# apache/horaedb

Measured on NVIDIA H100. Metric: scanned rows/s, higher is better.
Workload: dtype f64

## Files before the change

horaedb_b200/csrc/snappy.cu:

```cuda
#include "kernels.h"
#include "chunk_scratch.h"

#include <cstdlib>
#include <cstring>

#define SNP_FN __device__ __forceinline__
#define snp_shfl(v, src) __shfl_sync(0xffffffffu, (v), (src))
#define snp_shfl_up(v, d) __shfl_up_sync(0xffffffffu, (v), (d))
#define snp_ballot(p) __ballot_sync(0xffffffffu, (p))
#define snp_any(p) __any_sync(0xffffffffu, (p))
#define snp_syncwarp() __syncwarp()
#define snp_ldg8(p) __ldg(p)
#define snp_ldg64(p) __ldg(p)
#define snp_funnel_r(lo, hi, sh) __funnelshift_r((lo), (hi), (sh))
#define snp_byte_perm(a, b, s) __byte_perm((a), (b), (s))
#define snp_ffs(x) __ffs(x)
#define snp_set_err(err, code) atomicExch((err), (code))
namespace horae {
namespace snp {
__device__ __forceinline__ uint32_t snp_ldcg32(const uint32_t* p) {
  uint32_t v;
  asm volatile("ld.global.cg.u32 %0, [%1];" : "=r"(v) : "l"(p));
  return v;
}
__device__ __forceinline__ uint8_t snp_ldcg8(const uint8_t* p) {
  uint32_t v;
  asm volatile("ld.global.cg.u8 %0, [%1];" : "=r"(v) : "l"(p));
  return uint8_t(v);
}
}
}
#include "snappy_core.h"

namespace horae {
namespace k {

namespace {

using namespace horae::snp;
constexpr int kWarpsPerCta = 4;

__device__ __forceinline__ void init_tag_tables(uint8_t* s_csz, uint32_t* s_lut) {
  for (uint32_t t = threadIdx.x; t < 256; t += kWarpsPerCta * 32) { s_csz[t] = uint8_t(elem_csize(t)); s_lut[t] = elem_lut(t); }
  __syncthreads();
}

__global__ void __launch_bounds__(kWarpsPerCta * 32, 8) snappy_pages_kernel(const __grid_constant__ SnappyJob J) {
  __shared__ WarpSmem s_w[kWarpsPerCta];
  __shared__ uint32_t s_lut[256];
  __shared__ uint8_t s_csz[256];
  init_tag_tables(s_csz, s_lut);
  const int lane = threadIdx.x & 31, wid = threadIdx.x >> 5;
  WarpSmem& sm = s_w[wid];
  bulk_init(sm, lane);
  uint32_t phase = 0;
  const uint32_t nsel = J.d_nsel ? *J.d_nsel : J.nsel;
  const uint32_t nchunks = nsel * uint32_t(J.ncols);
  for (;;) {
    uint32_t c = 0;
    if (lane == 0) c = atomicAdd(J.ticket, 1u);
    c = __shfl_sync(0xffffffffu, c, 0);
    if (c >= nchunks) return;
    const uint32_t si = J.lpt ? J.lpt[c % nsel] : c % nsel;
    const int ci = J.order[c / nsel];
    RgSel rs = J.sel[si];
    SstDev sst = J.ssts[rs.sst];
    const ChunkDev* chunks = sst.chunks + size_t(rs.rg) * sst.ncols;
    ChunkDev ch = chunks[J.col_from_cols ? J.cols[ci].col : J.col[ci]];
    if (ch.codec != CODEC_SNAPPY) continue;
    if (ch.stored && J.skip_stored[ci]) continue;
    uint8_t* dst = J.scratch + (J.fixed_stride ? rs.scratch_off + uint64_t(J.region[ci]) * J.fixed_stride
                                               : chunk_scratch_off(rs, chunks, J.cols, ci));
    for (int p = ch.dict_uncomp ? -1 : 0; p < int(ch.num_pages); p++) {
      const uint8_t* src;
      uint32_t n, ulen, stop_at = 0xffffffffu;
      uint64_t advance;
      bool compressed = true;
      if (p < 0) {
        src = sst.bytes + ch.dict_payload_off; n = ch.dict_comp; ulen = ch.dict_uncomp;
        advance = dict_scratch(ch.codec, ch.phys, ch.dict_uncomp);
      } else {
        const PageDev pg = sst.pages[ch.first_page + p];
        const PageStream ps = page_stream(pg);
        src = sst.bytes + pg.payload_off + ps.skip; n = ps.comp; ulen = ps.out;
        compressed = ps.compressed;
        if (J.partial[ci]) {
          const uint32_t w = (ch.phys == 1 || ch.phys == 4) ? 4u : 8u;
          stop_at = 16u + (rs.num_rows + 7u) / 8u + 8u + rs.out_row * w;
        }
        advance = page_body_scratch(ch.codec, pg) + page_image_scratch(pg);
      }
      if (compressed) snappy_page(src, n, dst, ulen, stop_at, sm, phase, s_csz, s_lut, lane, J.err);
      dst += advance;
    }
  }
}

__global__ void __launch_bounds__(kWarpsPerCta * 32, 8) snappy_raw_kernel(const RawPage* __restrict__ pages, uint32_t n, unsigned int* ticket, int* err) {
  __shared__ WarpSmem s_w[kWarpsPerCta];
  __shared__ uint32_t s_lut[256];
  __shared__ uint8_t s_csz[256];
  init_tag_tables(s_csz, s_lut);
  const int lane = threadIdx.x & 31, wid = threadIdx.x >> 5;
  bulk_init(s_w[wid], lane);
  uint32_t phase = 0;
  for (;;) {
    uint32_t c = 0;
    if (lane == 0) c = atomicAdd(ticket, 1u);
    c = __shfl_sync(0xffffffffu, c, 0);
    if (c >= n) return;
    const RawPage pg = pages[c];
    snappy_page(pg.src, pg.comp_size, pg.dst, pg.uncomp_size, 0xffffffffu, s_w[wid], phase, s_csz, s_lut, lane, err);
  }
}

}

static uint32_t snappy_max_ctas() {
  static const int env = getenv("HORAE_SNAPPY_CTAS_PER_SM") ? atoi(getenv("HORAE_SNAPPY_CTAS_PER_SM")) : 0;
  int n = env > 0 ? env : 7;
  if (n > 8) n = 8;
  return uint32_t(kNumSMs) * uint32_t(n);
}

void snappy_raw_pages(const Launch& L, const RawPage* d_pages, uint32_t n, unsigned int* ticket, int* err) {
  if (!n) return;
  uint32_t ctas = (n + kWarpsPerCta - 1) / kWarpsPerCta;
  if (ctas > snappy_max_ctas()) ctas = snappy_max_ctas();
  snappy_raw_kernel<<<ctas, kWarpsPerCta * 32, 0, L.stream>>>(d_pages, n, ticket, err);
  L.tick();
}

void snappy_pages(const Launch& L, const SnappyJob& job, uint32_t max_chunks) {
  if (!max_chunks) return;
  uint32_t ctas = (max_chunks + kWarpsPerCta - 1) / kWarpsPerCta;
  if (ctas > snappy_max_ctas()) ctas = snappy_max_ctas();
  snappy_pages_kernel<<<ctas, kWarpsPerCta * 32, 0, L.stream>>>(job);
  L.tick();
}

void snappy_chunks(const Launch& L, const SstDev* ssts, const RgSel* sel, uint32_t nsel, const ColSel* cols, int ncolsel,
                   uint8_t* scratch, unsigned int* ticket, int* err) {
  if (!nsel || !ncolsel) return;
  SnappyJob J;
  std::memset(&J, 0, sizeof(J));
  J.ssts = ssts; J.sel = sel; J.d_nsel = nullptr; J.nsel = nsel; J.cols = cols; J.ncols = ncolsel;
  J.scratch = scratch; J.ticket = ticket; J.err = err; J.fixed_stride = 0;
  for (int i = 0; i < ncolsel && i < kSnappyMaxCols; i++) J.order[i] = uint8_t(i);
  J.col_from_cols = 1;
  snappy_pages(L, J, nsel * uint32_t(ncolsel));
}

}
}
```

horaedb_b200/csrc/snappy_core.h:

```cpp
#pragma once
#include <cstdint>

#ifndef SNP_STAT
#define SNP_STAT(counter, amount)
#endif

namespace horae {
namespace snp {

constexpr int kWin = 256;
constexpr int kWinPad = 16;
constexpr int kRing = 4096;
constexpr int kHist = 2048;
constexpr int kLevels = 5;
constexpr uint32_t kExit = 0xff;
constexpr uint32_t kRestage = kWin - 80;
constexpr uint32_t kFlushAt = 512;
constexpr uint64_t kFill = 0xfcfcfcfcfcfcfcfcull;

constexpr int kStage = 448;
constexpr uint32_t kAhead = kRestage;
struct alignas(256) WarpSmem {
  uint64_t ring64[kRing / 8];
  uint8_t J[kLevels][kWin];
  alignas(16) uint8_t stage[2][kStage];
  uint64_t bar[2];
};
constexpr uint32_t kJOff = kRing;
constexpr uint32_t kStageOff = kRing + kLevels * kWin;
constexpr uint32_t kBarOff = kStageOff + 2 * kStage;
struct StageState {
  uint32_t phase;
  int cur;
  bool pf;
  int pf_start;
  uint32_t pf_bytes;
};

SNP_FN uint32_t elem_csize(uint32_t t) {
  const uint32_t kind = t & 3;
  if (kind == 0) { const uint32_t l = t >> 2; return l < 60 ? l + 2 : 255u; }
  return kind == 1 ? 2u : (kind == 2 ? 3u : 5u);
}
SNP_FN uint32_t elem_lut(uint32_t t) {
  const uint32_t kind = t & 3;
  uint32_t len, hdr, offhi = 0, is_lit = 0, long_lit = 0, msh = 0;
  if (kind == 0) {
    const uint32_t l = t >> 2;
    is_lit = 1; hdr = 1;
    if (l < 60) len = l + 1; else { len = 0; long_lit = 1; }
  } else if (kind == 1) { len = ((t >> 2) & 7) + 4; hdr = 2; offhi = t >> 5; msh = 24; }
  else if (kind == 2) { len = (t >> 2) + 1; hdr = 3; msh = 16; }
  else { len = (t >> 2) + 1; hdr = 5; msh = 0; }
  const uint32_t csz = long_lit ? 0u : hdr + (is_lit ? len : 0u);
  return len | (offhi << 8) | (is_lit << 16) | (long_lit << 17) | (msh << 18) | (csz << 24);
}

SNP_FN uint64_t funnel64(uint64_t lo, uint64_t hi, uint32_t sh_bits) {
  return (lo >> sh_bits) | ((hi << 1) << (63 - sh_bits));
}
SNP_FN uint64_t ld8_any(const uint8_t* p) {
  const uintptr_t a = reinterpret_cast<uintptr_t>(p);
  const uint64_t* q = reinterpret_cast<const uint64_t*>(a & ~uintptr_t(7));
  return funnel64(snp_ldg64(q), snp_ldg64(q + 1), uint32_t(a & 7) * 8);
}
SNP_FN uint64_t ld8_out(const uint8_t* p) {
  const uintptr_t a = reinterpret_cast<uintptr_t>(p);
  const uint32_t* q = reinterpret_cast<const uint32_t*>(a & ~uintptr_t(3));
  const uint32_t sh = uint32_t(a & 3) * 8;
  const uint32_t x = snp_ldcg32(q), y = snp_ldcg32(q + 1), z = snp_ldcg32(q + 2);
  return (uint64_t(snp_funnel_r(y, z, sh)) << 32) | snp_funnel_r(x, y, sh);
}
SNP_FN uint8_t* ring_bytes(WarpSmem& sm) { return reinterpret_cast<uint8_t*>(sm.ring64); }
SNP_FN uint64_t ring_ld8(const WarpSmem& sm, uint32_t x) {
  const uint32_t w = (x >> 3) & (kRing / 8 - 1);
  return funnel64(sm.ring64[w], sm.ring64[(w + 1) & (kRing / 8 - 1)], (x & 7) * 8);
}
SNP_FN uint64_t sm_ld8(const WarpSmem& sm, uint32_t a) {
  const uint32_t* w = reinterpret_cast<const uint32_t*>(&sm) + (a >> 2);
  const uint32_t sh = (a & 3) * 8;
  const uint32_t x = w[0], y = w[1], z = w[2];
  return (uint64_t(snp_funnel_r(y, z, sh)) << 32) | snp_funnel_r(x, y, sh);
}
SNP_FN uint64_t shfl64(uint64_t v, int src) {
  const uint32_t lo = snp_shfl(uint32_t(v), src);
  const uint32_t hi = snp_shfl(uint32_t(v >> 32), src);
  return (uint64_t(hi) << 32) | lo;
}
template <int I> SNP_FN uint32_t byte_of(uint32_t x) { return snp_byte_perm(x, 0u, 0x4440u + I); }
template <int I> SNP_FN uint32_t put_byte(uint32_t acc, uint32_t v) {
  return snp_byte_perm(acc, v, I == 0 ? 0x3214u : (I == 1 ? 0x3240u : (I == 2 ? 0x3410u : 0x4210u)));
}

#ifdef __CUDACC__
template <int I, int LV> SNP_FN uint32_t jt_get(const WarpSmem&, uint32_t smbase, uint32_t packed) {
  uint32_t v;
  asm volatile("ld.shared.u8 %0, [%1+%2];" : "=r"(v) : "r"(__byte_perm(packed, smbase, 0x7650u + I)), "n"(kJOff + LV * kWin));
  return v;
}
SNP_FN uint32_t sm_base(const WarpSmem& sm) { return uint32_t(__cvta_generic_to_shared(&sm)); }
#define SNP_ST_BYTE(i, v) asm volatile("{ .reg .pred p; setp.gt.u32 p, %2, " #i "; @p st.shared.u8 [%0+" #i "], %1; }" ::"r"(a), "r"(v), "r"(len) : "memory")
SNP_FN void store_elem(WarpSmem&, uint32_t smbase, uint32_t rb, uint64_t w, uint32_t len) {
  const uint32_t a = smbase + rb, lo = uint32_t(w), hi = uint32_t(w >> 32);
  asm volatile("st.shared.u8 [%0], %1;" ::"r"(a), "r"(lo) : "memory");
  SNP_ST_BYTE(1, lo >> 8); SNP_ST_BYTE(2, lo >> 16); SNP_ST_BYTE(3, lo >> 24);
  SNP_ST_BYTE(4, hi); SNP_ST_BYTE(5, hi >> 8); SNP_ST_BYTE(6, hi >> 16); SNP_ST_BYTE(7, hi >> 24);
}
#undef SNP_ST_BYTE
#else
template <int I, int LV> SNP_FN uint32_t jt_get(const WarpSmem& sm, uint32_t, uint32_t packed) { return sm.J[LV][(packed >> (8 * I)) & 0xffu]; }
SNP_FN uint32_t sm_base(const WarpSmem&) { return 0; }
SNP_FN void store_elem(WarpSmem& sm, uint32_t, uint32_t rb, uint64_t w, uint32_t len) {
  for (uint32_t i = 0; i < len; i++) reinterpret_cast<uint8_t*>(sm.ring64)[rb + i] = uint8_t(w >> (8 * i));
}
#endif
#ifdef __CUDACC__
SNP_FN void bulk_init(WarpSmem& sm, int lane) {
  if (lane == 0) {
    const uint32_t a = sm_base(sm) + kBarOff;
    asm volatile("mbarrier.init.shared::cta.b64 [%0], 1;" ::"r"(a) : "memory");
    asm volatile("mbarrier.init.shared::cta.b64 [%0], 1;" ::"r"(a + 8) : "memory");
    asm volatile("fence.mbarrier_init.release.cluster;" ::: "memory");
  }
  snp_syncwarp();
}
SNP_FN void bulk_issue(WarpSmem& sm, int b, const uint8_t* g, uint32_t bytes, int lane) {
  if (lane == 0) {
    const uint32_t bar = sm_base(sm) + kBarOff + 8u * uint32_t(b), dst = sm_base(sm) + kStageOff + uint32_t(kStage) * uint32_t(b);
    asm volatile("fence.proxy.async.shared::cta;" ::: "memory");
    asm volatile("mbarrier.arrive.expect_tx.shared::cta.b64 _, [%0], %1;" ::"r"(bar), "r"(bytes) : "memory");
    asm volatile("cp.async.bulk.shared::cluster.global.mbarrier::complete_tx::bytes [%0], [%1], %2, [%3];" ::"r"(dst), "l"(g), "r"(bytes), "r"(bar) : "memory");
  }
}
SNP_FN void bulk_wait(WarpSmem& sm, int b, uint32_t parity) {
  const uint32_t bar = sm_base(sm) + kBarOff + 8u * uint32_t(b);
  uint32_t done;
  do {
    asm volatile("{ .reg .pred p; mbarrier.try_wait.parity.shared::cta.b64 p, [%1], %2; selp.u32 %0, 1, 0, p; }" : "=r"(done) : "r"(bar), "r"(parity) : "memory");
  } while (!done);
}
#else
SNP_FN void bulk_init(WarpSmem&, int) {}
SNP_FN void bulk_issue(WarpSmem& sm, int b, const uint8_t* g, uint32_t bytes, int lane) {
  if (lane == 0) for (uint32_t i = 0; i < bytes; i++) sm.stage[b][i] = g[i];
}
SNP_FN void bulk_wait(WarpSmem&, int, uint32_t) { snp_syncwarp(); }
#endif
SNP_FN void stage_fetch(WarpSmem& sm, StageState& st, int b, const uint8_t* src, uint32_t n, uint32_t from, int lane) {
  const uintptr_t a = reinterpret_cast<uintptr_t>(src + from) & ~uintptr_t(15);
  const uintptr_t end = (reinterpret_cast<uintptr_t>(src + n) + 15) & ~uintptr_t(15);
  uint32_t bytes = uint32_t(end - a);
  if (bytes > uint32_t(kStage)) bytes = uint32_t(kStage);
  st.pf_start = int(intptr_t(a) - intptr_t(reinterpret_cast<uintptr_t>(src)));
  st.pf_bytes = bytes;
  bulk_issue(sm, b, reinterpret_cast<const uint8_t*>(a), bytes, lane);
}

template <int LV> SNP_FN void jt_level(WarpSmem& sm, uint32_t smbase, uint32_t& jlo, uint32_t& jhi, int lane) {
  uint32_t nlo = 0, nhi = 0;
  nlo = put_byte<0>(nlo, jt_get<0, LV - 1>(sm, smbase, jlo)); nhi = put_byte<0>(nhi, jt_get<0, LV - 1>(sm, smbase, jhi));
  nlo = put_byte<1>(nlo, jt_get<1, LV - 1>(sm, smbase, jlo)); nhi = put_byte<1>(nhi, jt_get<1, LV - 1>(sm, smbase, jhi));
  nlo = put_byte<2>(nlo, jt_get<2, LV - 1>(sm, smbase, jlo)); nhi = put_byte<2>(nhi, jt_get<2, LV - 1>(sm, smbase, jhi));
  nlo = put_byte<3>(nlo, jt_get<3, LV - 1>(sm, smbase, jlo)); nhi = put_byte<3>(nhi, jt_get<3, LV - 1>(sm, smbase, jhi));
  jlo = nlo; jhi = nhi;
  reinterpret_cast<uint2*>(sm.J[LV])[lane] = make_uint2(jlo, jhi);
  snp_syncwarp();
}

SNP_FN void warp_copy_in(uint8_t* dst, const uint8_t* src, uint32_t len, int lane) {
  uint32_t head = uint32_t((8 - (reinterpret_cast<uintptr_t>(dst) & 7)) & 7);
  if (head > len) head = len;
  if (uint32_t(lane) < head) dst[lane] = snp_ldg8(src + lane);
  const uint32_t nwords = (len - head) >> 3;
  uint64_t* d8 = reinterpret_cast<uint64_t*>(dst + head);
  const uint8_t* s = src + head;
#pragma unroll 4
  for (uint32_t w = lane; w < nwords; w += 32) d8[w] = ld8_any(s + (size_t(w) << 3));
  const uint32_t done = head + (nwords << 3);
  for (uint32_t i = done + lane; i < len; i += 32) dst[i] = snp_ldg8(src + i);
}

SNP_FN uint8_t old_byte(WarpSmem& sm, const uint8_t* dst, uint32_t o, uint32_t x) {
  return (o - x <= uint32_t(kHist)) ? ring_bytes(sm)[x & (kRing - 1)] : snp_ldcg8(dst + x);
}

SNP_FN uint32_t flush_words(const WarpSmem& sm, uint8_t* dst, uint32_t fl, uint32_t upto, int lane) {
  const uint32_t w0 = fl >> 3, w1 = (upto >> 5) << 2;
  uint64_t* d8 = reinterpret_cast<uint64_t*>(dst);
  for (uint32_t w = w0 + lane; w < w1; w += 32) d8[w] = sm.ring64[w & (kRing / 8 - 1)];
  return w1 << 3;
}

SNP_FN void snappy_page_body(const uint8_t* __restrict__ src, uint32_t n, uint8_t* __restrict__ dst, uint32_t ulen_expected, uint32_t stop_at,
                             WarpSmem& sm, StageState& st, const uint8_t* __restrict__ csz, const uint32_t* __restrict__ lut, int lane, int* err) {
  uint32_t pos = 0, ulen = 0;
  for (int sh = 0; pos < n && sh < 35; sh += 7) {
    const uint32_t b = snp_ldg8(src + pos++);
    ulen |= (b & 0x7f) << sh;
    if (!(b & 0x80)) break;
  }
  if (ulen != ulen_expected) { if (lane == 0) snp_set_err(err, 101); return; }
  uint8_t* const ring = ring_bytes(sm);
  const uint32_t* const sm32 = reinterpret_cast<const uint32_t*>(&sm);
  const uint8_t* const sm8 = reinterpret_cast<const uint8_t*>(&sm);
  const uint32_t smbase = sm_base(sm);
  uint32_t o = 0;
  uint32_t fl = 0;
  while (pos < n && o < stop_at) {
    const uint32_t avail = n - pos;
    snp_syncwarp();
    SNP_STAT(windows, 1);
    uint32_t wbase;
    {
      const uint32_t need = avail < uint32_t(kWin + kWinPad) ? avail : uint32_t(kWin + kWinPad);
      const int nb = st.cur ^ 1;
      bool hit = false;
      if (st.pf) {
        bulk_wait(sm, nb, (st.phase >> nb) & 1u);
        st.phase ^= 1u << nb;
        st.pf = false;
        hit = int(pos) >= st.pf_start && pos + need <= uint32_t(st.pf_start + int(st.pf_bytes));
        SNP_STAT(stage_hits, hit ? 1 : 0);
      }
      if (!hit) {
        stage_fetch(sm, st, nb, src, n, pos, lane);
        bulk_wait(sm, nb, (st.phase >> nb) & 1u);
        st.phase ^= 1u << nb;
      }
      wbase = kStageOff + uint32_t(kStage) * uint32_t(nb) + uint32_t(int(pos) - st.pf_start);
      st.cur = nb;
      if (pos + kAhead < n) { stage_fetch(sm, st, nb ^ 1, src, n, pos + kAhead, lane); st.pf = true; }
    }
    const uint32_t tag0 = sm8[wbase];
    if ((tag0 & 3) == 0 && (tag0 >> 2) >= 60) {
      const uint32_t nb = (tag0 >> 2) - 59;
      uint32_t len = 0;
      for (uint32_t i = 0; i < nb && i + 1 < avail; i++) len |= uint32_t(sm8[wbase + 1 + i]) << (8 * i);
      len += 1;
      if (1 + nb > avail || o + len > ulen || len < 1) { if (lane == 0) snp_set_err(err, 102); return; }
      if (len > avail - 1 - nb) {
        if (o + (avail - 1 - nb) < stop_at) { if (lane == 0) snp_set_err(err, 102); return; }
        len = avail - 1 - nb;
      }
      const uint8_t* lsrc = src + pos + 1 + nb;
      snp_syncwarp();
      fl = flush_words(sm, dst, fl, o, lane);
      if (uint32_t(lane) < o - fl) dst[fl + lane] = ring[(fl + lane) & (kRing - 1)];
      warp_copy_in(dst + o, lsrc, len, lane);
      snp_syncwarp();
      const uint32_t keep = len < uint32_t(kHist) ? len : uint32_t(kHist);
      const uint32_t k0 = o + len - keep, k1 = o + len;
      const uint32_t a0 = (k0 + 7) & ~7u, a1 = k1 & ~7u;
      if (a0 < a1) {
        for (uint32_t w = (a0 >> 3) + lane; w < (a1 >> 3); w += 32) sm.ring64[w & (kRing / 8 - 1)] = ld8_any(lsrc + ((w << 3) - o));
        if (k0 + lane < a0) ring[(k0 + lane) & (kRing - 1)] = snp_ldg8(lsrc + (k0 + lane - o));
        if (a1 + lane < k1) ring[(a1 + lane) & (kRing - 1)] = snp_ldg8(lsrc + (a1 + lane - o));
      } else {
        for (uint32_t i = k0 + lane; i < k1; i += 32) ring[i & (kRing - 1)] = snp_ldg8(lsrc + (i - o));
      }
      snp_syncwarp();
      pos += 1 + nb + len;
      o += len;
      fl = o & ~31u;
      continue;
    }
    uint32_t jlo, jhi;
    {
      uint64_t w = kFill;
      const int nv = int(avail) - lane * 8;
      if (nv > 0) {
        w = sm_ld8(sm, wbase + uint32_t(lane) * 8);
        if (nv < 8) w = (w & ((1ull << (8 * nv)) - 1)) | (kFill << (8 * nv));
      }
      const uint32_t wl = uint32_t(w), wh = uint32_t(w >> 32), p0 = uint32_t(lane) * 8;
      uint32_t a;
      jlo = 0; jhi = 0;
      a = p0 + 0 + csz[byte_of<0>(wl)]; jlo = put_byte<0>(jlo, a < kExit ? a : kExit);
      a = p0 + 1 + csz[byte_of<1>(wl)]; jlo = put_byte<1>(jlo, a < kExit ? a : kExit);
      a = p0 + 2 + csz[byte_of<2>(wl)]; jlo = put_byte<2>(jlo, a < kExit ? a : kExit);
      a = p0 + 3 + csz[byte_of<3>(wl)]; jlo = put_byte<3>(jlo, a < kExit ? a : kExit);
      a = p0 + 4 + csz[byte_of<0>(wh)]; jhi = put_byte<0>(jhi, a < kExit ? a : kExit);
      a = p0 + 5 + csz[byte_of<1>(wh)]; jhi = put_byte<1>(jhi, a < kExit ? a : kExit);
      a = p0 + 6 + csz[byte_of<2>(wh)]; jhi = put_byte<2>(jhi, a < kExit ? a : kExit);
      a = p0 + 7 + csz[byte_of<3>(wh)]; jhi = put_byte<3>(jhi, a < kExit ? a : kExit);
      reinterpret_cast<uint2*>(sm.J[0])[lane] = make_uint2(jlo, jhi);
    }
    snp_syncwarp();
    jt_level<1>(sm, smbase, jlo, jhi, lane);
    jt_level<2>(sm, smbase, jlo, jhi, lane);
    jt_level<3>(sm, smbase, jlo, jhi, lane);
    jt_level<4>(sm, smbase, jlo, jhi, lane);
    uint32_t qs = 0;
    bool first = true;
    for (;;) {
      uint32_t q = qs;
#pragma unroll
      for (int lv = 0; lv < 5; lv++)
        if ((lane >> lv) & 1) q = sm.J[lv][q];
      const uint32_t e = lut[sm8[wbase + q]];
      uint32_t len = e & 0x7fu;
      uint32_t ecsz = e >> 24;
      bool is_lit = (e >> 16) & 1u;
      uint32_t off;
      {
        const uint32_t p1 = wbase + q + 1;
        const uint32_t raw = snp_funnel_r(sm32[p1 >> 2], sm32[(p1 >> 2) + 1], (p1 & 3) * 8);
        off = is_lit ? 0u : ((raw & (0xffffffffu >> ((e >> 18) & 31u))) | (e & 0x700u));
      }
      const bool valid = q != kExit && !((e >> 17) & 1u) && q + ecsz <= avail;
      const unsigned vm = snp_ballot(valid);
      const int m = (vm == 0xffffffffu) ? 32 : (snp_ffs(~vm) - 1);
      if (m == 0) {
        if (first) { if (lane == 0) snp_set_err(err, 105); return; }
        pos += qs;
        break;
      }
      first = false;
      if (lane >= m) { len = 0; ecsz = 0; off = 1; is_lit = true; }
      uint32_t inc = len;
#pragma unroll
      for (int d = 1; d < 32; d <<= 1) { const uint32_t t = snp_shfl_up(inc, d); if (lane >= d) inc += t; }
      const uint32_t doff = inc - len;
      {
        const bool bad = lane < m && !is_lit && (off == 0 || off > o + doff);
        if (snp_any(bad)) { if (lane == 0) snp_set_err(err, 103); return; }
      }
      const uint32_t len0 = snp_shfl(len, 0);
      int cnt;
      uint32_t T;
      if (len0 <= 8) {
        uint32_t skind = 0, spos = 0;
        bool fail = len > 8;
        const uint32_t s0 = doff - off;
        if (!is_lit && !fail) {
          if (off >= len) {
            if (s0 + len - 1 >= 0x80000000u) { skind = 1; spos = o + s0; }
            else if (s0 >= 0x80000000u) fail = true;
            else skind = 2;
          } else {
            if (doff == 0) { skind = 1; spos = o - off; } else fail = true;
          }
        }
        uint64_t w = 0;
        if (lane < m && !fail && skind != 2) {
          const uint32_t r = spos & (kRing - 1);
          if (skind == 1 && o - spos > uint32_t(kHist)) w = ld8_out(dst + spos);
          else if (skind == 1 && r > uint32_t(kRing) - 8) w = ring_ld8(sm, spos);
          else w = sm_ld8(sm, skind == 0 ? wbase + q + 1 : r);
          if (skind == 1 && off < len) {
            w &= (off >= 8) ? ~0ull : ((1ull << (8 * off)) - 1);
            for (uint32_t f = off; f < 8; f <<= 1) w |= w << (8 * f);
          }
        }
        uint32_t pp = uint32_t(lane);
        bool need = false;
        {
          const int cand = lane - int(off >> 2);
          const uint32_t x = snp_shfl(doff | (len << 16), cand);
          if (skind == 2) {
            const uint32_t d = s0 - (x & 0xffffu);
            if (cand >= 0 && cand < lane && d < 0x10000u && d + len <= (x >> 16)) pp = uint32_t(cand) | (d << 8);
            else need = true;
          }
        }
        if (snp_any(need)) {
          SNP_STAT(parent_searches, 1);
          int lo = 0;
#pragma unroll
          for (int step = 16; step > 0; step >>= 1) {
            const int cand = lo + step;
            const uint32_t d = snp_shfl(doff, cand & 31);
            if (need && cand < lane && d <= s0) lo = cand;
          }
          const uint32_t pd = snp_shfl(doff, lo), pl = snp_shfl(len, lo);
          if (need) {
            if (lo >= lane || s0 < pd || s0 + len > pd + pl) fail = true;
            else pp = uint32_t(lo) | ((s0 - pd) << 8);
          }
        }
        const unsigned fm = snp_ballot(fail || lane >= m);
        cnt = fm ? snp_ffs(fm) - 1 : 32;
        if (lane >= cnt) pp = uint32_t(lane);
#pragma unroll
        for (int it = 0; it < 5; it++) pp = snp_shfl(pp, int(pp)) + (pp & ~0xffu);
        {
          const uint64_t wr = shfl64(w, int(pp));
          if (skind == 2) w = wr >> (8 * (pp >> 8));
        }
        T = snp_shfl(inc, cnt - 1);
        if (o + T > ulen) { if (lane == 0) snp_set_err(err, 103); return; }
        if (lane < cnt) {
          const uint32_t rb = (o + doff) & (kRing - 1);
          if (rb <= uint32_t(kRing) - 8) store_elem(sm, smbase, rb, w, len);
          else {
#pragma unroll
            for (int i = 0; i < 8; i++)
              if (uint32_t(i) < len) ring[(rb + i) & (kRing - 1)] = uint8_t(w >> (8 * i));
          }
        }
      } else {
        const uint32_t off0 = snp_shfl(off, 0);
        const bool lit0 = snp_shfl(uint32_t(is_lit), 0) != 0;
        if (lit0) cnt = 1;
        else {
          const unsigned brk = snp_ballot(lane >= m || is_lit || off != off0);
          cnt = brk ? snp_ffs(brk) - 1 : 32;
        }
        T = snp_shfl(inc, cnt - 1);
        if (o + T > ulen) { if (lane == 0) snp_set_err(err, 103); return; }
        snp_syncwarp();
        if (lit0) {
          const uint32_t q0 = snp_shfl(q, 0);
          const uint8_t* ls = src + pos + q0 + 1;
          for (uint32_t i = lane; i < T; i += 32) ring[(o + i) & (kRing - 1)] = snp_ldg8(ls + i);
        } else if (off0 == 8 || off0 == 4 || off0 == 2 || off0 == 1) {
          uint64_t pw = ring_ld8(sm, o - off0);
          pw &= (off0 >= 8) ? ~0ull : ((1ull << (8 * off0)) - 1);
          for (uint32_t f = off0; f < 8; f <<= 1) pw |= pw << (8 * f);
          const uint32_t c = (off0 - (o % off0)) % off0;
          const uint64_t W = c ? ((pw >> (8 * c)) | (pw << (64 - 8 * c))) : pw;
          const uint32_t a0 = (o + 7) & ~7u, a1 = (o + T) & ~7u;
          if (a0 < a1) {
            for (uint32_t wd = (a0 >> 3) + lane; wd < (a1 >> 3); wd += 32) sm.ring64[wd & (kRing / 8 - 1)] = W;
            if (o + lane < a0) ring[(o + lane) & (kRing - 1)] = uint8_t(W >> (8 * ((o + lane) & 7)));
            if (a1 + lane < o + T) ring[(a1 + lane) & (kRing - 1)] = uint8_t(W >> (8 * lane));
          } else {
            for (uint32_t i = o + lane; i < o + T; i += 32) ring[i & (kRing - 1)] = uint8_t(W >> (8 * (i & 7)));
          }
        } else {
          const uint32_t stride = 32u % off0;
          uint32_t r = uint32_t(lane) % off0;
          for (uint32_t i = lane; i < T; i += 32) {
            const uint32_t x = o - off0 + r;
            ring[(o + i) & (kRing - 1)] = old_byte(sm, dst, o, x);
            r += stride;
            if (r >= off0) r -= off0;
          }
        }
      }
      snp_syncwarp();
      SNP_STAT(steps, 1); SNP_STAT(elements, cnt); SNP_STAT(word_steps, len0 <= 8 ? 1 : 0); SNP_STAT(bytes, T);
      o += T;
      if (o - fl >= kFlushAt) fl = flush_words(sm, dst, fl, o, lane);
      const uint32_t adv = snp_shfl(q + ecsz, cnt - 1);
      if (adv > kRestage || adv >= avail || o >= stop_at) { pos += adv; break; }
      qs = adv;
      snp_syncwarp();
    }
  }
  snp_syncwarp();
  fl = flush_words(sm, dst, fl, o, lane);
  if (fl + lane < o) dst[fl + lane] = ring[(fl + lane) & (kRing - 1)];
  if (o != ulen && o < stop_at) { if (lane == 0) snp_set_err(err, 104); }
}

SNP_FN void snappy_page(const uint8_t* __restrict__ src, uint32_t n, uint8_t* __restrict__ dst, uint32_t ulen_expected, uint32_t stop_at,
                        WarpSmem& sm, uint32_t& phase, const uint8_t* __restrict__ csz, const uint32_t* __restrict__ lut, int lane, int* err) {
  StageState st;
  st.phase = phase; st.cur = 0; st.pf = false; st.pf_start = 0; st.pf_bytes = 0;
  snappy_page_body(src, n, dst, ulen_expected, stop_at, sm, st, csz, lut, lane, err);
  snp_syncwarp();
  if (st.pf) {
    const int nb = st.cur ^ 1;
    bulk_wait(sm, nb, (st.phase >> nb) & 1u);
    st.phase ^= 1u << nb;
  }
  phase = st.phase;
}

}
}
```

Baseline: 46.23 billion.

## Add value-mode snappy fast path decoding literal+copy pairs as 8-byte values

For INT64/DOUBLE columns, adds a warp-wide fast path that treats each (short literal, 8-aligned copy) element pair as one 8-byte value per lane. It uses a sixth jump-table level to locate pairs and pointer-jumping over lanes to resolve dependencies, then writes whole 64-bit words to the ring. The general path also trims its batch so it does not split such pairs. This costs extra shared memory (one more jump level), which is why launch bounds drop from 8 to 7 CTAs per SM, plus an extra per-step check that is wasted when fewer than eight pairs qualify.

```diff
diff --git a/horaedb_b200/csrc/snappy.cu b/horaedb_b200/csrc/snappy.cu
--- a/horaedb_b200/csrc/snappy.cu
+++ b/horaedb_b200/csrc/snappy.cu
@@ -15,12 +15,18 @@
 #define snp_funnel_r(lo, hi, sh) __funnelshift_r((lo), (hi), (sh))
 #define snp_byte_perm(a, b, s) __byte_perm((a), (b), (s))
 #define snp_ffs(x) __ffs(x)
+#define SNP_HAVE_LDCG64 1
 #define snp_set_err(err, code) atomicExch((err), (code))
 namespace horae {
 namespace snp {
 __device__ __forceinline__ uint32_t snp_ldcg32(const uint32_t* p) {
   uint32_t v;
   asm volatile("ld.global.cg.u32 %0, [%1];" : "=r"(v) : "l"(p));
+  return v;
+}
+__device__ __forceinline__ uint64_t snp_ldcg64(const uint64_t* p) {
+  uint64_t v;
+  asm volatile("ld.global.cg.u64 %0, [%1];" : "=l"(v) : "l"(p));
   return v;
 }
 __device__ __forceinline__ uint8_t snp_ldcg8(const uint8_t* p) {
@@ -45,7 +51,7 @@
   __syncthreads();
 }
 
-__global__ void __launch_bounds__(kWarpsPerCta * 32, 8) snappy_pages_kernel(const __grid_constant__ SnappyJob J) {
+__global__ void __launch_bounds__(kWarpsPerCta * 32, 7) snappy_pages_kernel(const __grid_constant__ SnappyJob J) {
   __shared__ WarpSmem s_w[kWarpsPerCta];
   __shared__ uint32_t s_lut[256];
   __shared__ uint8_t s_csz[256];
@@ -71,6 +77,7 @@
     if (ch.stored && J.skip_stored[ci]) continue;
     uint8_t* dst = J.scratch + (J.fixed_stride ? rs.scratch_off + uint64_t(J.region[ci]) * J.fixed_stride
                                                : chunk_scratch_off(rs, chunks, J.cols, ci));
+    const bool vmode = ch.phys == PT_INT64 || ch.phys == PT_DOUBLE;
     for (int p = ch.dict_uncomp ? -1 : 0; p < int(ch.num_pages); p++) {
       const uint8_t* src;
       uint32_t n, ulen, stop_at = 0xffffffffu;
@@ -90,7 +97,7 @@
         }
         advance = page_body_scratch(ch.codec, pg) + page_image_scratch(pg);
       }
-      if (compressed) snappy_page(src, n, dst, ulen, stop_at, sm, phase, s_csz, s_lut, lane, J.err);
+      if (compressed) snappy_page(src, n, dst, ulen, stop_at, sm, phase, s_csz, s_lut, lane, J.err, vmode);
       dst += advance;
     }
   }
@@ -110,7 +117,7 @@
     c = __shfl_sync(0xffffffffu, c, 0);
     if (c >= n) return;
     const RawPage pg = pages[c];
-    snappy_page(pg.src, pg.comp_size, pg.dst, pg.uncomp_size, 0xffffffffu, s_w[wid], phase, s_csz, s_lut, lane, err);
+    snappy_page(pg.src, pg.comp_size, pg.dst, pg.uncomp_size, 0xffffffffu, s_w[wid], phase, s_csz, s_lut, lane, err, false);
   }
 }
 
diff --git a/horaedb_b200/csrc/snappy_core.h b/horaedb_b200/csrc/snappy_core.h
--- a/horaedb_b200/csrc/snappy_core.h
+++ b/horaedb_b200/csrc/snappy_core.h
@@ -3,6 +3,9 @@
 
 #ifndef SNP_STAT
 #define SNP_STAT(counter, amount)
+#endif
+#ifndef SNP_STAT_VALUE
+#define SNP_STAT_VALUE(amount)
 #endif
 
 namespace horae {
@@ -12,7 +15,8 @@
 constexpr int kWinPad = 16;
 constexpr int kRing = 4096;
 constexpr int kHist = 2048;
-constexpr int kLevels = 5;
+constexpr int kLevels = 6;
+constexpr int kMinValues = 8;
 constexpr uint32_t kExit = 0xff;
 constexpr uint32_t kRestage = kWin - 80;
 constexpr uint32_t kFlushAt = 512;
@@ -71,6 +75,20 @@
   const uint32_t x = snp_ldcg32(q), y = snp_ldcg32(q + 1), z = snp_ldcg32(q + 2);
   return (uint64_t(snp_funnel_r(y, z, sh)) << 32) | snp_funnel_r(x, y, sh);
 }
+SNP_FN uint64_t ldcg64(const uint64_t* q) {
+#ifdef SNP_HAVE_LDCG64
+  return snp_ldcg64(q);
+#else
+  const uint32_t* w = reinterpret_cast<const uint32_t*>(q);
+  return uint64_t(snp_ldcg32(w)) | (uint64_t(snp_ldcg32(w + 1)) << 32);
+#endif
+}
+SNP_FN uint64_t ld8_out64(const uint8_t* p) {
+  const uintptr_t a = reinterpret_cast<uintptr_t>(p);
+  const uint64_t* q = reinterpret_cast<const uint64_t*>(a & ~uintptr_t(7));
+  if (!(a & 7)) return ldcg64(q);
+  return funnel64(ldcg64(q), ldcg64(q + 1), uint32_t(a & 7) * 8);
+}
 SNP_FN uint8_t* ring_bytes(WarpSmem& sm) { return reinterpret_cast<uint8_t*>(sm.ring64); }
 SNP_FN uint64_t ring_ld8(const WarpSmem& sm, uint32_t x) {
   const uint32_t w = (x >> 3) & (kRing / 8 - 1);
@@ -192,7 +210,8 @@
 }
 
 SNP_FN void snappy_page_body(const uint8_t* __restrict__ src, uint32_t n, uint8_t* __restrict__ dst, uint32_t ulen_expected, uint32_t stop_at,
-                             WarpSmem& sm, StageState& st, const uint8_t* __restrict__ csz, const uint32_t* __restrict__ lut, int lane, int* err) {
+                             bool vmode, WarpSmem& sm, StageState& st, const uint8_t* __restrict__ csz, const uint32_t* __restrict__ lut,
+                             int lane, int* err) {
   uint32_t pos = 0, ulen = 0;
   for (int sh = 0; pos < n && sh < 35; sh += 7) {
     const uint32_t b = snp_ldg8(src + pos++);
@@ -290,9 +309,81 @@
     jt_level<2>(sm, smbase, jlo, jhi, lane);
     jt_level<3>(sm, smbase, jlo, jhi, lane);
     jt_level<4>(sm, smbase, jlo, jhi, lane);
+    if (vmode) jt_level<5>(sm, smbase, jlo, jhi, lane);
     uint32_t qs = 0;
     bool first = true;
     for (;;) {
+      if (vmode) {
+        uint32_t qv = qs;
+#pragma unroll
+        for (int lv = 0; lv < 5; lv++)
+          if ((lane >> lv) & 1) qv = sm.J[lv + 1][qv];
+        const uint32_t el = lut[sm8[wbase + qv]];
+        const uint32_t L = el & 0x7fu, lcsz = el >> 24;
+        const uint32_t qc = qv + (lcsz < 5u ? lcsz : 5u);
+        const uint32_t ec = lut[sm8[wbase + qc]];
+        const uint32_t ccsz = ec >> 24;
+        uint32_t lit4, off;
+        {
+          const uint32_t p1 = wbase + qv + 1, p2 = wbase + qc + 1;
+          lit4 = snp_funnel_r(sm32[p1 >> 2], sm32[(p1 >> 2) + 1], (p1 & 3) * 8);
+          const uint32_t raw = snp_funnel_r(sm32[p2 >> 2], sm32[(p2 >> 2) + 1], (p2 & 3) * 8);
+          off = (raw & (0xffffffffu >> ((ec >> 18) & 31u))) | (ec & 0x700u);
+        }
+        const uint32_t k8 = uint32_t(lane) * 8;
+        const bool ok = qv != kExit && ((el >> 16) & 3u) == 1u && L <= 4u && !((ec >> 16) & 1u) && (ec & 0x7fu) == 8u - L &&
+                        off != 0 && !(off & 7u) && off <= o + k8 && qc + ccsz <= avail && o + k8 + 8 <= ulen;
+        const unsigned okm = snp_ballot(ok);
+        const int cv = (okm == 0xffffffffu) ? 32 : (snp_ffs(~okm) - 1);
+        if (cv >= kMinValues) {
+          const bool in = uint32_t(lane) < uint32_t(cv);
+          const uint32_t back = off >> 3;
+          const bool old = in && back > uint32_t(lane);
+          uint64_t w = 0;
+          const uint32_t ph = o & 7u;
+          if (old) {
+            const uint32_t x = o + k8 - off;
+            if (off - k8 > uint32_t(kHist)) w = ld8_out64(dst + x);
+            else w = ph ? ring_ld8(sm, x) : sm.ring64[(x >> 3) & (kRing / 8 - 1)];
+            const uint64_t lm = (1ull << (8 * L)) - 1;
+            w = (w & ~lm) | (uint64_t(lit4) & lm);
+          }
+          uint32_t s = uint32_t(lane);
+          if (in) s = (old ? uint32_t(lane) : uint32_t(lane) - back) | (L << 5) | (lit4 & uint32_t((1ull << (8 * L)) - 1) & 0xffffff00u);
+#pragma unroll
+          for (int it = 0; it < 5; it++) {
+            const uint32_t t = snp_shfl(s, int(s & 31u));
+            const uint32_t l1 = (s >> 5) & 7u, l2 = (t >> 5) & 7u;
+            const uint32_t mine = uint32_t((1ull << (8 * l1)) - 1);
+            s = (t & 31u) | ((l1 > l2 ? l1 : l2) << 5) | (((s & mine) | (t & ~mine)) & 0xffffff00u);
+          }
+          const uint32_t lk = (s >> 5) & 7u;
+          const uint64_t root = shfl64(w, int(s & 31u));
+          const uint64_t v = (root & (~0ull << (8 * lk))) | (s & 0xffffff00u) | (lit4 & 0xffu);
+          const uint32_t wb = o >> 3;
+          if (!ph) {
+            if (in) sm.ring64[(wb + uint32_t(lane)) & (kRing / 8 - 1)] = v;
+          } else {
+            const uint32_t sh = 8 * ph;
+            uint64_t prev = (uint64_t(snp_shfl_up(uint32_t(v >> 32), 1)) << 32) | snp_shfl_up(uint32_t(v), 1);
+            uint64_t lo = prev >> (64 - sh);
+            if (lane == 0) lo = sm.ring64[wb & (kRing / 8 - 1)] & ((1ull << sh) - 1);
+            if (in) sm.ring64[(wb + uint32_t(lane)) & (kRing / 8 - 1)] = lo | (v << sh);
+            if (lane == cv - 1) sm.ring64[(wb + uint32_t(lane) + 1) & (kRing / 8 - 1)] = v >> (64 - sh);
+          }
+          snp_syncwarp();
+          const uint32_t T = uint32_t(cv) * 8;
+          SNP_STAT(steps, 1); SNP_STAT_VALUE(1); SNP_STAT(elements, 2 * cv); SNP_STAT(bytes, T);
+          first = false;
+          o += T;
+          if (o - fl >= kFlushAt) fl = flush_words(sm, dst, fl, o, lane);
+          const uint32_t adv = snp_shfl(qc + ccsz, cv - 1);
+          if (adv > kRestage || adv >= avail || o >= stop_at) { pos += adv; break; }
+          qs = adv;
+          snp_syncwarp();
+          continue;
+        }
+      }
       uint32_t q = qs;
 #pragma unroll
       for (int lv = 0; lv < 5; lv++)
@@ -380,6 +471,14 @@
         }
         const unsigned fm = snp_ballot(fail || lane >= m);
         cnt = fm ? snp_ffs(fm) - 1 : 32;
+        if (vmode) {
+          const uint32_t nx = snp_shfl(len | (uint32_t(!is_lit && off != 0 && !(off & 7u)) << 8), (lane + 1) & 31);
+          const bool pair = lane < 31 && is_lit && len <= 4u && nx == (8u - len) + 0x100u;
+          const bool cand = pair && 2 * lane >= cnt && lane < cnt;
+          const unsigned pm = snp_ballot(cand);
+          const unsigned last = snp_ballot(cand && (pm >> lane) == 1u);
+          if (last) cnt = snp_ffs(last) - 1;
+        }
         if (lane >= cnt) pp = uint32_t(lane);
 #pragma unroll
         for (int it = 0; it < 5; it++) pp = snp_shfl(pp, int(pp)) + (pp & ~0xffu);
@@ -455,10 +554,11 @@
 }
 
 SNP_FN void snappy_page(const uint8_t* __restrict__ src, uint32_t n, uint8_t* __restrict__ dst, uint32_t ulen_expected, uint32_t stop_at,
-                        WarpSmem& sm, uint32_t& phase, const uint8_t* __restrict__ csz, const uint32_t* __restrict__ lut, int lane, int* err) {
+                        WarpSmem& sm, uint32_t& phase, const uint8_t* __restrict__ csz, const uint32_t* __restrict__ lut, int lane, int* err,
+                        bool vmode = false) {
   StageState st;
   st.phase = phase; st.cur = 0; st.pf = false; st.pf_start = 0; st.pf_bytes = 0;
-  snappy_page_body(src, n, dst, ulen_expected, stop_at, sm, st, csz, lut, lane, err);
+  snappy_page_body(src, n, dst, ulen_expected, stop_at, vmode, sm, st, csz, lut, lane, err);
   snp_syncwarp();
   if (st.pf) {
     const int nb = st.cur ^ 1;
```

Measured after the change: 51.20 billion (median of 6 runs). +10.8%, better.
